# jason-gideon/GPUMounter

Measured on AMD Instinct MI355X. Metric: p50_gpu_attach_latency_ms, lower is better.
Workload: dtype none

## Files before the change

### gpumounter_amd/_native.py

```python
from __future__ import annotations

import ctypes as C
import os
import subprocess
import threading
from typing import Optional

LIB_DIR = os.path.join(os.path.dirname(os.path.abspath(__file__)), "_lib")
NATIVE_DIR = os.path.join(os.path.dirname(os.path.dirname(os.path.abspath(__file__))), "native")

_lock = threading.Lock()
_libs: dict = {}


class NativeError(RuntimeError):
    pass


def lib_path(name: str) -> str:
    return os.path.join(LIB_DIR, name)


def build(target: str = "all", quiet: bool = True) -> None:
    import fcntl
# ... 71 lines not shown
def mock_smi() -> C.CDLL:
    lib = _load("libamd_smi_mock.so", "host")
    lib.gm_mock_set_procs_file.argtypes = [C.c_char_p]
    lib.gm_mock_set_ecc.argtypes = [C.c_uint32, C.c_uint64, C.c_uint64]
    return lib


class DevRule(C.Structure):
    _fields_ = [("type", C.c_char), ("access", C.c_uint8), ("allow", C.c_uint8),
                ("pad", C.c_uint8), ("major", C.c_int32), ("minor", C.c_int32)]


class DevNode(C.Structure):
    _fields_ = [("path", C.c_char * 112), ("major", C.c_uint32), ("minor", C.c_uint32),
                ("mode", C.c_uint32), ("uid", C.c_int32), ("gid", C.c_int32)]


class BpfTiming(C.Structure):
    _fields_ = [("query_ns", C.c_uint64), ("map_ns", C.c_uint64), ("build_ns", C.c_uint64),
                ("load_ns", C.c_uint64), ("attach_ns", C.c_uint64), ("programs", C.c_uint32),
                ("insns", C.c_uint32)]


HOST_ABI_VERSION = 6
GM_ACC_MKNOD, GM_ACC_READ, GM_ACC_WRITE = 1, 2, 4
GM_DEV_EMULATE, GM_DEV_VIA_SETNS, GM_DEV_REPLACE, GM_DEV_BIND = 1, 2, 4, 8


def host() -> C.CDLL:
    lib = _load("libgm_host.so", "host")
    if not getattr(lib, "_gm_typed", False):
        abi = lib.gm_host_abi_version()
        if abi != HOST_ABI_VERSION:
            raise RuntimeError(f"libgm_host.so ABI {abi} != {HOST_ABI_VERSION} expected: stale "
                               f"build, run `make -C native`")
        lib.gm_cg1_apply.argtypes = [C.c_char_p, C.POINTER(DevRule), C.c_int]
        lib.gm_cg1_format_rule.argtypes = [C.POINTER(DevRule), C.c_char_p, C.c_int]
        lib.gm_bpf_dev_build.argtypes = [C.POINTER(DevRule), C.c_int, C.c_int, C.c_int,
                                         C.POINTER(C.c_uint64), C.c_int]
        lib.gm_bpf_dev_load.argtypes = [C.POINTER(C.c_uint64), C.c_int, C.c_char_p, C.c_char_p,
                                        C.c_int]
        lib.gm_bpf_dev_query.argtypes = [C.c_char_p, C.POINTER(C.c_uint32), C.c_uint32,
                                         C.POINTER(C.c_uint32), C.POINTER(C.c_uint32)]
        lib.gm_bpf_prog_name.argtypes = [C.c_uint32, C.c_char_p, C.c_int]
        lib.gm_bpf_dev_program.argtypes = [C.c_char_p, C.POINTER(C.c_uint64), C.c_uint32,
                                           C.POINTER(C.c_uint32), C.POINTER(C.c_uint32)]
        lib.gm_bpf_dev_program_at.argtypes = [C.c_char_p, C.c_uint32, C.c_int,
                                              C.POINTER(C.c_uint64),
                                              C.c_uint32, C.POINTER(C.c_uint32),
# ... 3 lines not shown
                                           C.POINTER(C.c_uint32), C.POINTER(C.c_uint32)]
        lib.gm_bpf_dev_restore.argtypes = [C.c_char_p, C.c_char_p]
        lib.gm_bpf_dev_build_set.argtypes = [C.c_int, C.POINTER(DevRule), C.c_int, C.c_int,
                                             C.c_int, C.POINTER(C.c_uint64), C.c_int]
        lib.gm_bpf_dev_probe_set.argtypes = []
        lib.gm_devnodes_bind_probe.argtypes = []
        lib.gm_bpf_dev_straight_line.argtypes = [C.c_int]
        lib.gm_bpf_dev_straight_line.restype = None
        lib.gm_bpf_dev_set_at.argtypes = [C.c_char_p, C.c_uint32, C.POINTER(C.c_uint32),
                                          C.c_uint32, C.POINTER(C.c_uint32),
                                          C.POINTER(C.c_uint32)]
        lib.gm_bpf_dev_last_timing.argtypes = [C.POINTER(BpfTiming)]
        lib.gm_bpf_dev_last_timing.restype = None
        lib.gm_devnodes_create.argtypes = [C.c_int, C.c_char_p, C.POINTER(DevNode), C.c_int,
                                           C.c_int, C.POINTER(C.c_int)]
        lib.gm_devnodes_remove.argtypes = lib.gm_devnodes_create.argtypes
        lib.gm_devnodes_guard.argtypes = [C.c_char_p]
        lib.gm_devnodes_stage.argtypes = [C.c_char_p, C.c_int]
        lib.gm_devnode_stat.argtypes = [C.c_int, C.c_char_p, C.c_char_p, C.c_int,
                                        C.POINTER(C.c_int), C.POINTER(C.c_uint32),
                                        C.POINTER(C.c_uint32), C.POINTER(C.c_uint32)]
        lib.gm_devnodes_present.argtypes = [C.c_int, C.c_char_p, C.POINTER(DevNode), C.c_int,
                                            C.c_int, C.POINTER(C.c_uint8)]
        lib.gm_proc_dev_users.argtypes = [C.c_uint32, C.c_uint32, C.POINTER(C.c_int32), C.c_int,
                                          C.POINTER(C.c_int)]
        lib.gm_proc_scan_devs.argtypes = [C.POINTER(C.c_int32), C.c_int, C.POINTER(C.c_uint32),
                                          C.c_int, C.POINTER(C.c_uint8), C.POINTER(C.c_int32)]
        lib.gm_proc_filter_dev_users.argtypes = [C.POINTER(C.c_int32), C.c_int, C.c_uint32,
                                                 C.c_uint32, C.POINTER(C.c_int32)]
        lib.gm_proc_read_pids.argtypes = [C.c_char_p, C.POINTER(C.c_int32), C.c_int,
                                          C.POINTER(C.c_int)]
        lib.gm_sd_get_device_allow.argtypes = [C.c_char_p, C.c_char_p, C.c_char_p, C.c_int,
                                               C.c_char_p, C.c_int]
        lib.gm_sd_set_device_allow.argtypes = [C.c_char_p, C.c_char_p, C.POINTER(C.c_char_p),
                                               C.POINTER(C.c_char_p), C.c_int, C.c_int,
                                               C.c_char_p, C.c_int]
        lib.gm_sd_unit_path.argtypes = [C.c_char_p, C.c_char_p, C.c_int]
        lib.gm_roctx_push.argtypes = [C.c_char_p]
        lib.gm_roctx_mark.argtypes = [C.c_char_p]
        lib.gm_roctx_start.argtypes = [C.c_char_p]
        lib.gm_roctx_start.restype = C.c_uint64
        lib.gm_roctx_stop.argtypes = [C.c_uint64]
        lib.gm_roctx_stop.restype = None
        lib.gm_now_ns.restype = C.c_uint64
        lib._gm_typed = True
    return lib
# ... 113 lines not shown
```

### gpumounter_amd/node/devnodes.py

```python
from __future__ import annotations

import ctypes as C
import errno
import os
from dataclasses import dataclass
from typing import List, Optional, Sequence, Tuple

from gpumounter_amd import _native
from gpumounter_amd.models.device import DeviceNode
from gpumounter_amd.utils import log


class DevNodeError(RuntimeError):
    def __init__(self, msg: str, results: Sequence[int] = ()):
        super().__init__(msg)
        self.results = list(results)


@dataclass(frozen=True)
class Target:

    pid: int = 0
    root: str = ""

# ... 6 lines not shown
class DevNodeWriter:

    def __init__(self, mode: str = "procroot", host_dev: str = "", userns: str = "auto",
                 stage_dir: str = "", proc_root: str = "/proc") -> None:
        self.mode = mode
        self.userns = userns
        self.stage_dir = stage_dir
        self.proc_root = proc_root
        self._staged = False
        self._own_userns = self._userns_id("self")
        self.flags = 0
        if mode == "setns":
            self.flags |= _native.GM_DEV_VIA_SETNS
        if mode == "emulate":
            self.flags |= _native.GM_DEV_EMULATE
        self.host_dev = host_dev
        rc = _native.host().gm_devnodes_guard(host_dev.encode() if host_dev else None)
        if rc < 0:
            _log.warning("host /dev guard off: cannot read %s (%s)", host_dev, os.strerror(-rc))
        self.guarded = max(rc, 0)

    @staticmethod
    def _array(nodes: Sequence[DeviceNode], owner: Tuple[int, int] = (-1, -1)):
        arr = (_native.DevNode * max(len(nodes), 1))()
        for i, n in enumerate(nodes):
            rel = n.path.lstrip("/").encode()
            if len(rel) >= 112:
                raise DevNodeError(f"path too long: {n.path}")
            arr[i].path = rel
            arr[i].major = n.major
            arr[i].minor = n.minor
            arr[i].mode = n.mode
            arr[i].uid, arr[i].gid = owner
        return arr

    def _mntns(self, pid) -> Optional[str]:
        try:
            return os.readlink(f"{self.proc_root}/{pid}/ns/mnt")
        except OSError:
            return None

    def root_pid(self, pids: Sequence[int]) -> int:
        if self.mode == "emulate":
            return pids[0] if pids else 0
        own = self._mntns("self")
        for pid in pids:
            ns = self._mntns(pid)
            if ns is not None and ns != own:
                return pid
        return 0

    def _userns_id(self, pid) -> Optional[Tuple[int, int]]:
        try:
            st = os.stat(f"{self.proc_root}/{pid}/ns/user")
        except OSError:
            return None
        return st.st_dev, st.st_ino
# ... 43 lines not shown
        if not self._bind(t):
            return self.flags, (-1, -1)
        self._ensure_stage()
        return self.flags | _native.GM_DEV_BIND, self._mapped_root(t)

    def _target_args(self, t: Target) -> Tuple[int, Optional[bytes]]:
        if t.root:
            return 0, t.root.encode()
        if t.pid <= 0:
            raise DevNodeError("container has no process to resolve its root from "
                               "(empty cgroup.procs)")
        return t.pid, None

    def create(self, t: Target, nodes: Sequence[DeviceNode]) -> List[int]:
        if not nodes:
            return []
        pid, root = self._target_args(t)
        flags, owner = self._call(t)
        res = (C.c_int * len(nodes))()
        fails = _native.host().gm_devnodes_create(pid, root, self._array(nodes, owner),
                                                  len(nodes), flags, res)
        results = [int(res[i]) for i in range(len(nodes))]
        if fails:
            bad = [(n.path, os.strerror(-r)) for n, r in zip(nodes, results) if r < 0]
            what = "bind mount" if flags & _native.GM_DEV_BIND else "mknod"
            raise DevNodeError(f"{what} failed: {bad}", results)
        return results

    def remove(self, t: Target, nodes: Sequence[DeviceNode]) -> List[int]:
        if not nodes:
            return []
        pid, root = self._target_args(t)
        flags, _ = self._call(t)
        res = (C.c_int * len(nodes))()
        fails = _native.host().gm_devnodes_remove(pid, root, self._array(nodes), len(nodes),
                                                  flags, res)
        results = [int(res[i]) for i in range(len(nodes))]
        if fails and not flags & _native.GM_DEV_BIND and \
                any(r == -errno.EBUSY for r in results) and self.mode != "emulate":
            busy = [i for i, r in enumerate(results) if r == -errno.EBUSY]
            self._ensure_stage()
            sub = [nodes[i] for i in busy]
            res2 = (C.c_int * len(sub))()
            _native.host().gm_devnodes_remove(pid, root, self._array(sub), len(sub),
                                              flags | _native.GM_DEV_BIND, res2)
            for k, i in enumerate(busy):
                results[i] = int(res2[k])
            fails = sum(1 for r in results if r < 0)
        if fails:
            if all(r in (-errno.ESRCH, -errno.ENOENT) for r in results if r < 0):
# ... 37 lines not shown
```

### gpumounter_amd/node/hotmount.py

```python
from __future__ import annotations

import os
from dataclasses import dataclass, field
from typing import Dict, List, Optional, Sequence

from gpumounter_amd.hw.inventory import Inventory
from gpumounter_amd.models.device import AmdGpu, DeviceNode, kfd_node
from gpumounter_amd.models.pod import ContainerRef, running_containers
from gpumounter_amd.node.cgroup import CgroupError, CgroupResolver, DeviceRuleBackend
from gpumounter_amd.node.devnodes import CREATED, DevNodeError, DevNodeWriter, Target
from gpumounter_amd.node.journal import InjectionJournal
from gpumounter_amd.utils import log, trace

_log = log.get("node.hotmount")


class MountError(RuntimeError):
    pass


@dataclass
class ContainerTarget:
    ref: ContainerRef
    cgdir: str
    target: Target
    pids: List[int] = field(default_factory=list)


@dataclass
class AuditIssue:
    container: str
    kind: str
    path: str
    major: int
    minor: int


class HotMount:
    def __init__(self, cfg, inv: Inventory, resolver: CgroupResolver, backend: DeviceRuleBackend,
                 writer: DevNodeWriter, faults=None,
                 journal: Optional[InjectionJournal] = None) -> None:
        from gpumounter_amd.utils.faults import NONE

        self.cfg = cfg
        self.inv = inv
        self.resolver = resolver
        self.backend = backend
        self.writer = writer
        self.faults = faults if faults is not None else NONE
        self.journal = journal if journal is not None else InjectionJournal()
        self.expected: Dict[str, object] = {}

    def _apply(self, cgdir: str, grant, revoke, desired) -> None:
        try:
            self.backend.apply(cgdir, grant, revoke, desired)
        finally:
            fp = getattr(self.backend, "fingerprint", None)
            self.expected[cgdir] = fp(cgdir) if fp is not None else None

    def kfd(self) -> DeviceNode:
        return kfd_node(self.inv.kfd_major)

    def gpu_nodes(self, gpus: Sequence[AmdGpu]) -> List[DeviceNode]:
        out: List[DeviceNode] = []
        for g in sorted(gpus, key=lambda g: g.index):
            out.extend(g.device_nodes(self.cfg.drm_major, self.cfg.inject_card_nodes,
                                      self.cfg.device_file_mode))
        return out

    def managed_nodes(self, hot: Sequence[AmdGpu], base: Sequence[AmdGpu]) -> List[DeviceNode]:
        base_keys = {(n.major, n.minor) for n in self.gpu_nodes(base)}
        nodes = [n for n in self.gpu_nodes(hot) if (n.major, n.minor) not in base_keys]
        if hot and not base:
            nodes.insert(0, self.kfd())
# ... 20 lines not shown

    def _owner(self, pod: dict, t: ContainerTarget) -> dict:
        md = pod.get("metadata", {})
        return {"namespace": md.get("namespace", ""), "pod": md.get("name", ""),
                "pod_uid": md.get("uid", ""), "container": t.ref.name, "cgdir": t.cgdir}

    def resolve(self, pod: dict, container: str = "",
                include_privileged: bool = False) -> List[ContainerTarget]:
        try:
            return self.targets(pod, container, include_privileged)
        except (CgroupError, OSError) as e:
            raise MountError(f"cannot resolve the pod's containers: {e}") from e

    def attach(self, pod: dict, new: Sequence[AmdGpu], have: Sequence[AmdGpu],
               base: Sequence[AmdGpu] = (), container: str = "") -> List[ContainerTarget]:
        before = self.managed_nodes(have, base)
        after = self.managed_nodes(list(have) + list(new), base)
        before_keys = {(n.major, n.minor) for n in before}
        grant = [n for n in after if (n.major, n.minor) not in before_keys]
        with trace.span("resolve"):
            targets = self.resolve(pod, container)
        done: List[tuple] = []
        j = self.journal
        try:
            for t in targets:
                cid = t.ref.id
                known = j.nodes_of(cid)
                with trace.span("devnodes_probe", nodes=len(after)):
                    states = self.writer.present_states(t.target, after)
                theirs = {(n.major, n.minor) for n, st in zip(after, states)
                          if st and (n.major, n.minor) not in known}
                j.intend(cid, [((n.major, n.minor), n.path) for n in grant],
                         [((n.major, n.minor), n.path) for n in after
                          if (n.major, n.minor) not in theirs], **self._owner(pod, t))
                done.append((t, grant, []))
                with trace.span("cgroup_rule", backend=self.backend.name, rules=len(grant)):
                    self.faults.check("cgroup_rule")
                    self._apply(t.cgdir, grant, [], after)
                self.faults.check("cgroup_rule", "after")
                with trace.span("devnodes", nodes=len(after)):
                    self.faults.check("devnodes")
                    res = self.writer.create(t.target, after)
                done[-1] = (t, grant, [n for n, r in zip(after, res) if r == CREATED])
                j.settle(cid, [(n.major, n.minor) for n, r in zip(after, res)
                               if r != CREATED and (n.major, n.minor) not in known
                               and (n.major, n.minor) not in theirs])
                self.faults.check("devnodes", "after")
        except Exception as e:
            self._rollback_attach(done, before)
            for t in targets[len(done):]:
                self._forget_new(t.ref.id, grant, after, before)
            raise MountError(f"attach failed, rolled back: {e}") from e
        return targets

    def _forget_new(self, cid: str, granted, after, before) -> None:
        keep = {(n.major, n.minor) for n in before}
        self.journal.forget(cid, [(n.major, n.minor) for n in granted],
                            [(n.major, n.minor) for n in after if (n.major, n.minor) not in keep])

    def _rollback_attach(self, done, before: List[DeviceNode]) -> None:
        before_keys = {(n.major, n.minor) for n in before}
        for t, granted, created in reversed(done):
            try:
                self.writer.remove(t.target, created)
            except Exception as e:
                _log.error("rollback unlink in %s failed: %s", t.ref.name, e)
            else:
                self.journal.forget(t.ref.id, (), [(n.major, n.minor) for n in created
                                                   if (n.major, n.minor) not in before_keys])
            try:
                try:
                    have = self.backend.installed(t.cgdir)
                    revoke = [n for n in granted if (n.major, n.minor) in have]
                except Exception:
                    revoke = list(granted)
                if revoke:
                    self._apply(t.cgdir, [], revoke, before)
            except Exception as e:
                _log.error("rollback revoke in %s failed: %s", t.cgdir, e)
            else:
                self.journal.forget(t.ref.id, [(n.major, n.minor) for n in granted])
            ent = self.journal.nodes_of(t.ref.id)
            self.journal.forget(t.ref.id, (), [k for k in ent if k not in before_keys])

    def detach(self, pod: dict, remove: Sequence[AmdGpu], keep: Sequence[AmdGpu],
               base: Sequence[AmdGpu] = (), container: str = "",
               targets: Optional[List[ContainerTarget]] = None) -> List[ContainerTarget]:
        before = self.managed_nodes(list(keep) + list(remove), base)
        after = self.managed_nodes(keep, base)
        after_keys = {(n.major, n.minor) for n in after}
        revoke = [n for n in before if (n.major, n.minor) not in after_keys]
        if targets is None:
            with trace.span("resolve"):
                targets = self.resolve(pod, container)
        try:
            self._detach(targets, revoke, after)
        except (CgroupError, DevNodeError, OSError) as e:
            raise MountError(f"detach failed: {e}") from e
        return targets

    def _detach(self, targets: List[ContainerTarget], revoke: List[DeviceNode],
                after: List[DeviceNode]) -> None:
        keys = [(n.major, n.minor) for n in revoke]
        for t in targets:
            with trace.span("cgroup_rule", backend=self.backend.name, rules=len(revoke)):
                self.faults.check("unmount")
                self._apply(t.cgdir, [], revoke, after)
            self.faults.check("unmount", "after")
            ours = self.journal.nodes_of(t.ref.id)
            unlink = [n for n in revoke if (n.major, n.minor) in ours]
            with trace.span("devnodes", nodes=len(unlink)):
                self.writer.remove(t.target, unlink)
            self.journal.forget(t.ref.id, keys, keys)

    def adopt(self, pod: dict, hot: Sequence[AmdGpu], base: Sequence[AmdGpu] = ()) -> int:
        want = self.managed_nodes(hot, base)
        if not want:
            return 0
        n = 0
        for t in self.targets(pod):
            if self.journal.get(t.ref.id) is not None:
                continue
            granted = self.backend.installed(t.cgdir)
            states = self.writer.present_states(t.target, want)
            rules = [((d.major, d.minor), d.path) for d in want if (d.major, d.minor) in granted]
            nodes = [((d.major, d.minor), d.path) for d, st in zip(want, states) if st == 1]
            if rules or nodes:
# ... 122 lines not shown
```

### gpumounter_amd/node/journal.py

```python
from __future__ import annotations

import json
import os
import threading
import time
from dataclasses import dataclass, field
from typing import Dict, Iterable, List, Optional, Tuple

from gpumounter_amd.utils import log

_log = log.get("node.journal")

Key = Tuple[int, int]


@dataclass
class Entry:
    container_id: str
    namespace: str = ""
    pod: str = ""
    pod_uid: str = ""
    container: str = ""
    cgdir: str = ""
    rules: Dict[Key, str] = field(default_factory=dict)
    nodes: Dict[Key, str] = field(default_factory=dict)
    updated: float = 0.0

    def empty(self) -> bool:
        return not self.rules and not self.nodes

    def to_json(self) -> dict:
        return {"container_id": self.container_id, "namespace": self.namespace, "pod": self.pod,
                "pod_uid": self.pod_uid, "container": self.container, "cgdir": self.cgdir,
                "rules": sorted([ma, mi, p] for (ma, mi), p in self.rules.items()),
                "nodes": sorted([ma, mi, p] for (ma, mi), p in self.nodes.items()),
                "updated": self.updated}
# ... 80 lines not shown
    def _entry(self, cid: str, owner: Optional[dict]) -> Entry:
        if not _safe_id(cid):
            raise ValueError(f"journal: bad container id {cid!r}")
        e = self._entries.get(cid)
        if e is None:
            e = self._entries[cid] = Entry(cid)
        if owner:
            for k, v in owner.items():
                if v:
                    setattr(e, k, v)
        return e

    def intend(self, cid: str, rules: Iterable[Tuple[Key, str]] = (),
               nodes: Iterable[Tuple[Key, str]] = (), **owner: str) -> None:
        with self._mu:
            e = self._entry(cid, owner)
            before = (len(e.rules), len(e.nodes))
            e.rules.update(rules)
            e.nodes.update(nodes)
            if (len(e.rules), len(e.nodes)) != before or not e.updated:
                e.updated = time.time()
                self._store(e)

    def settle(self, cid: str, not_ours: Iterable[Key]) -> None:
        keys = list(not_ours)
        if not keys:
            return
        with self._mu:
            e = self._entries.get(cid)
            if e is None:
                return
            changed = False
            for k in keys:
                changed |= e.nodes.pop(k, None) is not None
            if changed:
                e.updated = time.time()
                self._store(e)

    def forget(self, cid: str, rules: Iterable[Key] = (), nodes: Iterable[Key] = ()) -> None:
        with self._mu:
            e = self._entries.get(cid)
            if e is None:
                return
            changed = False
            for k in rules:
                changed |= e.rules.pop(k, None) is not None
# ... 16 lines not shown
```

### gpumounter_amd/utils/trace.py

```python
from __future__ import annotations

import contextvars
import os
import threading
import time
from dataclasses import dataclass, field
from typing import Callable, Dict, List, Optional

_current: contextvars.ContextVar[Optional["Span"]] = contextvars.ContextVar("gm_span", default=None)

_roctx_lock = threading.Lock()
_roctx = None
_sinks: List[Callable[["Span"], None]] = []


_names: Dict[str, bytes] = {}


def _profiled() -> bool:
    mode = os.environ.get("GM_ROCTX", "auto").lower()
    if mode in ("on", "1", "true"):
        return True
    if mode in ("off", "0", "false"):
        return False
# ... 83 lines not shown
        self.s.start_ns = time.perf_counter_ns()
        return self.s

    def __exit__(self, et, ev, tb):
        self.s.end_ns = time.perf_counter_ns()
        if ev is not None:
            self.s.error = f"{et.__name__}: {ev}"
        if self._lib is not None:
            self._lib.gm_roctx_stop(self._rid)
        _current.reset(self._tok)
        if self.s.parent is None:
            for fn in list(_sinks):
                try:
                    fn(self.s)
                except Exception:
                    pass
        return False


def current() -> Optional[Span]:
    return _current.get()


def record(name: str, duration_ns: int, **attrs) -> None:
    parent = _current.get()
    if parent is None or duration_ns <= 0:
        return
    start = parent.children[-1].end_ns if parent.children and parent.children[-1].end_ns \
        else parent.start_ns
    parent.children.append(Span(name=name, start_ns=start, end_ns=start + int(duration_ns),
                                attrs=attrs, parent=parent))


def annotate(**attrs) -> None:
    s = _current.get()
    if s is not None:
        s.attrs.update(attrs)


def mark(name: str) -> None:
    lib = _roctx_lib()
    if lib is not None:
        lib.gm_roctx_mark(name.encode())
```

### native/include/gm_host.h

```cpp
#pragma once
#include <stdint.h>

#ifdef __cplusplus
extern "C" {
#endif

#define GM_HOST_ABI_VERSION 6

#define GM_ACC_MKNOD 1
#define GM_ACC_READ 2
#define GM_ACC_WRITE 4

typedef struct gm_dev_rule {
  char type;
  uint8_t access;
  uint8_t allow;
  uint8_t pad;
  int32_t major;
  int32_t minor;
} gm_dev_rule_t;

int gm_cg1_apply(const char* cgdir, const gm_dev_rule_t* rules, int n);
int gm_cg1_format_rule(const gm_dev_rule_t* rule, char* out, int cap);

int gm_bpf_dev_build(const gm_dev_rule_t* rules, int n, int default_allow, int chain_map_fd,
                     uint64_t* out, int cap);
int gm_bpf_dev_build_set(int set_map_fd, const gm_dev_rule_t* base, int nbase, int default_allow,
                         int chain_map_fd, uint64_t* out, int cap);
int gm_bpf_dev_load(const uint64_t* insns, int n, const char* name, char* log, int logcap);
int gm_bpf_dev_query(const char* cgroup_path, uint32_t* ids, uint32_t cap, uint32_t* n,
// ... 24 lines not shown
  uint32_t minor;
  uint32_t mode;
  int32_t uid;
  int32_t gid;
} gm_dev_node_t;

#define GM_DEV_EMULATE 1
#define GM_DEV_VIA_SETNS 2
#define GM_DEV_REPLACE 4
#define GM_DEV_BIND 8

int gm_devnodes_guard(const char* host_dev);
int gm_devnodes_stage(const char* dir, int mount_tmpfs);
int gm_devnodes_bind_probe(void);
int gm_devnodes_create(int pid, const char* root, const gm_dev_node_t* nodes, int n, int flags,
                       int* results);
int gm_devnodes_remove(int pid, const char* root, const gm_dev_node_t* nodes, int n, int flags,
                       int* results);
int gm_devnode_stat(int pid, const char* root, const char* path, int flags, int* kind,
                    uint32_t* major, uint32_t* minor, uint32_t* mode);
int gm_devnodes_present(int pid, const char* root, const gm_dev_node_t* nodes, int n, int flags,
                        uint8_t* present);

int gm_proc_dev_users(uint32_t major, uint32_t minor, int32_t* pids, int cap, int* n);
int gm_proc_scan_devs(const int32_t* pids, int n, const uint32_t* majmin, int ndev,
                      uint8_t* hits, int32_t* unreadable);
int gm_proc_filter_dev_users(const int32_t* pids, int n, uint32_t major, uint32_t minor,
                             int32_t* out);
int gm_proc_read_pids(const char* path, int32_t* pids, int cap, int* n);

int gm_sd_get_device_allow(const char* bus_path, const char* unit, char* out, int cap, char* err,
                           int errcap);
int gm_sd_set_device_allow(const char* bus_path, const char* unit, const char* const* paths,
                           const char* const* perms, int n, int reset, char* err, int errcap);
int gm_sd_unit_path(const char* unit, char* out, int cap);

int gm_roctx_available(void);
void gm_roctx_push(const char* name);
void gm_roctx_pop(void);
void gm_roctx_mark(const char* name);
uint64_t gm_roctx_start(const char* name);
void gm_roctx_stop(uint64_t id);
uint64_t gm_now_ns(void);

int gm_host_abi_version(void);

// ... 4 lines not shown
```

### native/src/gm_host.cpp

```cpp
#include "gm_host.h"

#include <dirent.h>
#include <dlfcn.h>
#include <errno.h>
#include <fcntl.h>
#include <linux/bpf.h>
#include <sched.h>
#include <signal.h>
#include <stdio.h>
#include <stdlib.h>
#include <string.h>
#include <sys/mount.h>
#include <sys/stat.h>
#include <sys/syscall.h>
#include <sys/sysmacros.h>
#include <time.h>
#include <unistd.h>

#include <atomic>
#include <map>
#include <mutex>
#include <string>
#include <thread>
#include <vector>
// ... 502 lines not shown
  }
  if (comps.empty()) return -EINVAL;
  int cur = dup(rootfd);
  if (cur < 0) return -errno;
  Fd curfd(cur);
  for (size_t i = 0; i + 1 < comps.size(); ++i) {
    int nfd = openat(curfd.fd, comps[i].c_str(), O_PATH | O_DIRECTORY | O_NOFOLLOW | O_CLOEXEC);
    if (nfd < 0 && errno == ENOENT && create) {
      if (guarded_dir(curfd.fd)) return kSharedHost;
      if (mkdirat(curfd.fd, comps[i].c_str(), 0755) < 0 && errno != EEXIST) return -errno;
      nfd = openat(curfd.fd, comps[i].c_str(), O_PATH | O_DIRECTORY | O_NOFOLLOW | O_CLOEXEC);
    }
    if (nfd < 0) return -errno;
    curfd = Fd(nfd);
  }
  *leaf = comps.back();
  *parent = std::move(curfd);
  return 0;
}

struct Walker {
  int rootfd;
  bool mknod_denied = false;
  std::map<std::string, Fd> dirs;
  explicit Walker(int r) : rootfd(r) {}
  int parent(const char* path, bool create, int* dirfd, std::string* leaf) {
    std::string p(path);
    size_t cut = p.rfind('/');
    std::string dir = cut == std::string::npos ? std::string() : p.substr(0, cut);
    auto it = dirs.find(dir);
    if (it != dirs.end()) {
      *leaf = p.substr(cut + 1);
      if (leaf->empty() || *leaf == "." || *leaf == "..") return -EINVAL;
      *dirfd = it->second.fd;
      return 0;
    }
    Fd fd;
    int e = walk_parent(rootfd, path, create, &fd, leaf);
    if (e != 0) return e;
    *dirfd = fd.fd;
    dirs.emplace(dir, std::move(fd));
    return 0;
  }
};

int stat_leaf(int dirfd, const std::string& leaf, int* kind, uint32_t* maj, uint32_t* min,
              uint32_t* mode) {
  struct stat st;
  *kind = 0;
  *maj = *min = *mode = 0;
  if (fstatat(dirfd, leaf.c_str(), &st, AT_SYMLINK_NOFOLLOW) < 0) {
    if (errno == ENOENT) return 0;
    return -errno;
  }
  *mode = st.st_mode & 07777;
  if (S_ISCHR(st.st_mode)) {
    *kind = 1;
    *maj = major(st.st_rdev);
    *min = minor(st.st_rdev);
    return 0;
  }
  *kind = 3;
// ... 841 lines not shown
  if (e < 0) {
    for (int i = 0; i < n; ++i) results[i] = e;
    return n;
  }
  return failures;
}

int gm_devnode_stat(int pid, const char* root, const char* path, int flags, int* kind,
                    uint32_t* maj, uint32_t* min, uint32_t* mode) {
  return with_root(pid, root, flags, [&](int rootfd) {
    Fd parent;
    std::string leaf;
    int e = walk_parent(rootfd, path, false, &parent, &leaf);
    if (e == -ENOENT) {
      *kind = 0;
      *maj = *min = *mode = 0;
      return 0;
    }
    if (e < 0) return e;
    return stat_leaf(parent.fd, leaf, kind, maj, min, mode);
  });
}

int gm_devnodes_present(int pid, const char* root, const gm_dev_node_t* nodes, int n, int flags,
                        uint8_t* present) {
  int count = 0;
  int e = with_root(pid, root, flags, [&](int rootfd) {
    Walker wk(rootfd);
    for (int i = 0; i < n; ++i) {
      present[i] = 0;
      int pfd;
      std::string leaf;
      int w = wk.parent(nodes[i].path, false, &pfd, &leaf);
      if (w == -ENOENT) {
        std::string dir(nodes[i].path);
        const size_t cut = dir.rfind('/');
        dir = cut == std::string::npos ? std::string() : dir.substr(0, cut);
        Fd d2;
        std::string l2;
        if (!dir.empty() && walk_parent(rootfd, dir.c_str(), false, &d2, &l2) == 0 &&
            guarded_dir(d2.fd)) {
          present[i] = kSharedHost;
          ++count;
        }
        continue;
      }
      if (w < 0) continue;
      if (guarded_dir(pfd)) {
        present[i] = kSharedHost;
        ++count;
        continue;
      }
      int kind = 0;
      uint32_t ma = 0, mi = 0, mode = 0;
      if (stat_leaf(pfd, leaf, &kind, &ma, &mi, &mode) < 0) continue;
      if ((kind == 1 || kind == 2) && ma == nodes[i].major && mi == nodes[i].minor &&
          (!(flags & GM_DEV_BIND) || is_mount_leaf(pfd, leaf) == 1)) {
        present[i] = 1;
        ++count;
      }
    }
    return 0;
  });
  return e < 0 ? e : count;
}

namespace {
bool pid_uses_dev(long pid, dev_t want) {
  char p[64];
  snprintf(p, sizeof(p), "/proc/%ld/fd", pid);
  int dfd = open(p, O_RDONLY | O_DIRECTORY | O_CLOEXEC);
  if (dfd < 0) return false;
  DIR* fds = fdopendir(dfd);
  if (!fds) {
    close(dfd);
    return false;
  }
  struct dirent* fe;
  bool hit = false;
  while (!hit && (fe = readdir(fds)) != nullptr) {
    if (fe->d_name[0] == '.') continue;
    struct stat st;
    if (fstatat(dirfd(fds), fe->d_name, &st, 0) == 0 && S_ISCHR(st.st_mode) && st.st_rdev == want)
      hit = true;
  }
  closedir(fds);
  return hit;
// ... 110 lines not shown
```

Baseline: 1.091.

## Fuse attach/detach probe, journal, cgroup rule and node creation into one native transaction

Result: no change. 1.101 (+1.0%).

```diff
diff --git a/gpumounter_amd/_native.py b/gpumounter_amd/_native.py
--- a/gpumounter_amd/_native.py
+++ b/gpumounter_amd/_native.py
@@ -117,9 +117,28 @@
                 ("insns", C.c_uint32)]
 
 
-HOST_ABI_VERSION = 6
+class Txn(C.Structure):
+    _fields_ = [("pid", C.c_int32), ("flags", C.c_int32), ("root", C.c_char_p),
+                ("desired", C.POINTER(DevNode)), ("known", C.POINTER(C.c_uint8)),
+                ("unlink", C.POINTER(DevNode)), ("n_desired", C.c_int32),
+                ("n_unlink", C.c_int32), ("cgdir", C.c_char_p), ("pin_dir", C.c_char_p),
+                ("base", C.POINTER(DevRule)), ("n_base", C.c_int32), ("backend", C.c_int32),
+                ("journal_path", C.c_char_p), ("record", C.c_char_p),
+                ("record_len", C.c_int32), ("fp_cap", C.c_int32),
+                ("states", C.POINTER(C.c_uint8)), ("results", C.POINTER(C.c_int32)),
+                ("fp", C.c_void_p), ("fp_len", C.c_int32), ("stage", C.c_int32),
+                ("err", C.c_int32), ("dir_walks", C.c_int32), ("prog_id", C.c_uint32),
+                ("chained_id", C.c_uint32), ("probe_ns", C.c_uint64),
+                ("journal_ns", C.c_uint64), ("rule_ns", C.c_uint64), ("nodes_ns", C.c_uint64)]
+
+
+HOST_ABI_VERSION = 7
 GM_ACC_MKNOD, GM_ACC_READ, GM_ACC_WRITE = 1, 2, 4
 GM_DEV_EMULATE, GM_DEV_VIA_SETNS, GM_DEV_REPLACE, GM_DEV_BIND = 1, 2, 4, 8
+GM_TXN_RECORDING, GM_TXN_BPF_SET = 1, 2
+(GM_TXN_ARGS, GM_TXN_PROBE, GM_TXN_JOURNAL, GM_TXN_RULE, GM_TXN_NODES,
+ GM_TXN_DONE) = range(6)
+GM_TXN_FOREIGN_NODE = 1
 
 
 def host() -> C.CDLL:
@@ -169,6 +188,8 @@
                                         C.POINTER(C.c_uint32), C.POINTER(C.c_uint32)]
         lib.gm_devnodes_present.argtypes = [C.c_int, C.c_char_p, C.POINTER(DevNode), C.c_int,
                                             C.c_int, C.POINTER(C.c_uint8)]
+        lib.gm_hotmount_attach.argtypes = [C.POINTER(Txn)]
+        lib.gm_hotmount_detach.argtypes = [C.POINTER(Txn)]
         lib.gm_proc_dev_users.argtypes = [C.c_uint32, C.c_uint32, C.POINTER(C.c_int32), C.c_int,
                                           C.POINTER(C.c_int)]
         lib.gm_proc_scan_devs.argtypes = [C.POINTER(C.c_int32), C.c_int, C.POINTER(C.c_uint32),
diff --git a/gpumounter_amd/node/devnodes.py b/gpumounter_amd/node/devnodes.py
--- a/gpumounter_amd/node/devnodes.py
+++ b/gpumounter_amd/node/devnodes.py
@@ -52,17 +52,14 @@
 
     @staticmethod
     def _array(nodes: Sequence[DeviceNode], owner: Tuple[int, int] = (-1, -1)):
-        arr = (_native.DevNode * max(len(nodes), 1))()
-        for i, n in enumerate(nodes):
+        uid, gid = owner
+        init = []
+        for n in nodes:
             rel = n.path.lstrip("/").encode()
             if len(rel) >= 112:
                 raise DevNodeError(f"path too long: {n.path}")
-            arr[i].path = rel
-            arr[i].major = n.major
-            arr[i].minor = n.minor
-            arr[i].mode = n.mode
-            arr[i].uid, arr[i].gid = owner
-        return arr
+            init.append((rel, n.major, n.minor, n.mode, uid, gid))
+        return (_native.DevNode * max(len(nodes), 1))(*init)
 
     def _mntns(self, pid) -> Optional[str]:
         try:
@@ -152,10 +149,15 @@
                                                   len(nodes), flags, res)
         results = [int(res[i]) for i in range(len(nodes))]
         if fails:
-            bad = [(n.path, os.strerror(-r)) for n, r in zip(nodes, results) if r < 0]
-            what = "bind mount" if flags & _native.GM_DEV_BIND else "mknod"
-            raise DevNodeError(f"{what} failed: {bad}", results)
+            raise self.create_error(nodes, results, flags)
         return results
+
+    @staticmethod
+    def create_error(nodes: Sequence[DeviceNode], results: Sequence[int],
+                     flags: int = 0) -> DevNodeError:
+        bad = [(n.path, os.strerror(-r)) for n, r in zip(nodes, results) if r < 0]
+        what = "bind mount" if flags & _native.GM_DEV_BIND else "mknod"
+        return DevNodeError(f"{what} failed: {bad}", results)
 
     def remove(self, t: Target, nodes: Sequence[DeviceNode]) -> List[int]:
         if not nodes:
diff --git a/gpumounter_amd/node/hotmount.py b/gpumounter_amd/node/hotmount.py
--- a/gpumounter_amd/node/hotmount.py
+++ b/gpumounter_amd/node/hotmount.py
@@ -1,14 +1,20 @@
 from __future__ import annotations
 
+import ctypes as C
+import errno
 import os
 from dataclasses import dataclass, field
 from typing import Dict, List, Optional, Sequence
 
+from gpumounter_amd import _native
 from gpumounter_amd.hw.inventory import Inventory
 from gpumounter_amd.models.device import AmdGpu, DeviceNode, kfd_node
 from gpumounter_amd.models.pod import ContainerRef, running_containers
-from gpumounter_amd.node.cgroup import CgroupError, CgroupResolver, DeviceRuleBackend
-from gpumounter_amd.node.devnodes import CREATED, DevNodeError, DevNodeWriter, Target
+from gpumounter_amd.node.cgroup import (BPF_STATE, CgroupError, CgroupResolver,
+                                        DeviceRuleBackend, V2BpfBackend, V2RecordingBackend,
+                                        _rule_array, oci_default_rules)
+from gpumounter_amd.node.devnodes import (CREATED, SHARED_HOST, DevNodeError, DevNodeWriter,
+                                          Target)
 from gpumounter_amd.node.journal import InjectionJournal
 from gpumounter_amd.utils import log, trace
 
@@ -50,6 +56,8 @@
         self.faults = faults if faults is not None else NONE
         self.journal = journal if journal is not None else InjectionJournal()
         self.expected: Dict[str, object] = {}
+        self.txn_counts: Dict[str, int] = {"fused": 0, "stepwise": 0}
+        self._txn_base = None
 
     def _apply(self, cgdir: str, grant, revoke, desired) -> None:
         try:
@@ -116,8 +124,12 @@
             targets = self.resolve(pod, container)
         done: List[tuple] = []
         j = self.journal
+        arr = self._txn_nodes(after) if self._fusable() else None
         try:
             for t in targets:
+                if arr is not None and self._attach_fused(pod, t, grant, after, arr, done):
+                    continue
+                self.txn_counts["stepwise"] += 1
                 cid = t.ref.id
                 known = j.nodes_of(cid)
                 with trace.span("devnodes_probe", nodes=len(after)):
@@ -152,6 +164,173 @@
         self.journal.forget(cid, [(n.major, n.minor) for n in granted],
                             [(n.major, n.minor) for n in after if (n.major, n.minor) not in keep])
 
+    _WRITER_STEPS = frozenset(("present_states", "create", "remove"))
+    _BACKEND_STEPS = frozenset(("apply", "fingerprint"))
+    _JOURNAL_STEPS = frozenset(("intend", "settle", "forget", "nodes_of"))
+
+    def _fusable(self) -> bool:
+        if self.faults:
+            return False
+        b, w, j = self.backend, self.writer, self.journal
+        if not (type(b) is V2RecordingBackend or (type(b) is V2BpfBackend and b.set_mode)):
+            return False
+        if type(w) is not DevNodeWriter or w.mode not in ("procroot", "emulate") \
+                or type(j) is not InjectionJournal:
+            return False
+        return self._WRITER_STEPS.isdisjoint(vars(w)) and \
+            self._BACKEND_STEPS.isdisjoint(vars(b)) and self._JOURNAL_STEPS.isdisjoint(vars(j))
+
+    def _txn_nodes(self, nodes: Sequence[DeviceNode]):
+        if any(n.path[:1] != "/" or n.path[1:2] == "/" for n in nodes):
+            return None
+        try:
+            return self.writer._array(nodes)
+        except DevNodeError:
+            return None
+
+    def _txn(self, t: ContainerTarget, after: Sequence[DeviceNode], arr, touch_root: bool):
+        w = self.writer
+        x = _native.Txn()
+        x.flags = w.flags
+        if touch_root:
+            try:
+                x.pid, x.root = w._target_args(t.target)
+                x.flags = w._call(t.target)[0]
+            except DevNodeError:
+                return None
+            if x.flags & _native.GM_DEV_BIND:
+                return None
+        n = len(after)
+        x.desired, x.n_desired = arr, n
+        x.cgdir = t.cgdir.encode()
+        if type(self.backend) is V2RecordingBackend:
+            x.backend = _native.GM_TXN_RECORDING
+            cap = 2048 + 192 * n
+        else:
+            x.backend = _native.GM_TXN_BPF_SET
+            x.pin_dir = self.backend.pin_dir.encode() if self.backend.pin_dir else None
+            if self._txn_base is None:
+                base = oci_default_rules()
+                self._txn_base = (_rule_array(base), len(base))
+            x.base, x.n_base = self._txn_base
+            cap = 64
+        x._fp = C.create_string_buffer(cap)
+        x.fp, x.fp_cap = C.addressof(x._fp), cap
+        j = self.journal
+        x.journal_path = j._path(t.ref.id).encode() if j.dir else None
+        return x
+
+    def _txn_rule_effects(self, x, cgdir: str, rules: int,
+                          desired: Sequence[DeviceNode]) -> None:
+        b = self.backend
+        ok = x.stage > _native.GM_TXN_RULE
+        b._installed.pop(cgdir, None)
+        if x.backend == _native.GM_TXN_RECORDING:
+            fp = C.string_at(x.fp, x.fp_len) if x.fp_len >= 0 else None
+            if ok and desired and fp is not None:
+                b._installed[cgdir] = (fp, frozenset((d.major, d.minor) for d in desired))
+        else:
+            fp = None if x.fp_len < 0 else \
+                tuple(C.cast(x.fp, C.POINTER(C.c_uint32))[i] for i in range(x.fp_len // 4))
+        self.expected[cgdir] = fp
+        sp = trace.record("cgroup_rule", x.rule_ns, backend=b.name, rules=rules)
+        if x.backend == _native.GM_TXN_BPF_SET and ok and desired:
+            if sp is not None:
+                tm = _native.BpfTiming()
+                _native.host().gm_bpf_dev_last_timing(C.byref(tm))
+                trace.record("bpf_query", tm.query_ns, sp)
+                trace.record("bpf_build", tm.build_ns, sp, insns=tm.insns)
+                trace.record("bpf_load_verify", tm.load_ns, sp, programs=tm.programs)
+                trace.record("bpf_chain_map", tm.map_ns, sp)
+                trace.record("bpf_attach", tm.attach_ns, sp)
+            log.kv(_log, 10, "bpf program installed", cgroup=cgdir, prog_id=x.prog_id,
+                   chained=x.chained_id, rules=x.n_desired)
+
+    def _txn_rule_error(self, x, cgdir: str) -> Exception:
+        msg = os.strerror(-x.err)
+        if x.backend == _native.GM_TXN_RECORDING:
+            return OSError(-x.err, msg, os.path.join(cgdir, BPF_STATE))
+        what = "install" if x.n_desired else "restore"
+        return CgroupError(f"bpf {what} on {cgdir}: {msg}")
+
+    def _attach_fused(self, pod: dict, t: ContainerTarget, grant: List[DeviceNode],
+                      after: List[DeviceNode], arr, done: List[tuple]) -> bool:
+        n = len(after)
+        x = self._txn(t, after, arr, touch_root=n > 0)
+        if x is None:
+            return False
+        j = self.journal
+        cid = t.ref.id
+        known = j.nodes_of(cid)
+        ent, blob = j.stage_intend(cid, [((d.major, d.minor), d.path) for d in grant],
+                                   [((d.major, d.minor), d.path) for d in after],
+                                   **self._owner(pod, t))
+        x.record, x.record_len = blob, len(blob or b"")
+        x._known = (C.c_uint8 * max(n, 1))(*[(d.major, d.minor) in known for d in after])
+        x._states = (C.c_uint8 * max(n, 1))()
+        x._results = (C.c_int32 * max(n, 1))()
+        x.known, x.states, x.results = x._known, x._states, x._results
+        rc = _native.host().gm_hotmount_attach(C.byref(x))
+        if rc == _native.GM_TXN_FOREIGN_NODE or x.stage == _native.GM_TXN_ARGS \
+                or (x.stage == _native.GM_TXN_RULE and x.err == -errno.ENOSPC):
+            return False
+        self.txn_counts["fused"] += 1
+        if x.stage == _native.GM_TXN_PROBE:
+            raise DevNodeError(f"read-back of {n} nodes: {os.strerror(-x.err)}")
+        trace.record("devnodes_probe", x.probe_ns, nodes=n)
+        j.adopt(ent, blob is not None, keep_empty=True)
+        if x.stage == _native.GM_TXN_JOURNAL:
+            raise OSError(-x.err, os.strerror(-x.err), j._path(cid))
+        done.append((t, grant, []))
+        self._txn_rule_effects(x, t.cgdir, len(grant), after)
+        if x.stage == _native.GM_TXN_RULE:
+            raise self._txn_rule_error(x, t.cgdir)
+        trace.record("devnodes", x.nodes_ns, nodes=n)
+        res = [int(x._results[i]) for i in range(n)]
+        if x.stage == _native.GM_TXN_NODES:
+            raise self.writer.create_error(after, res, x.flags)
+        done[-1] = (t, grant, [d for d, r in zip(after, res) if r == CREATED])
+        j.settle(cid, [(d.major, d.minor) for d, r in zip(after, res)
+                       if r != CREATED and (d.major, d.minor) not in known])
+        return True
+
+    def _detach_fused(self, t: ContainerTarget, revoke: List[DeviceNode],
+                      after: List[DeviceNode], arr, keys: List[tuple]) -> bool:
+        j = self.journal
+        cid = t.ref.id
+        ours = j.nodes_of(cid)
+        unlink = [d for d in revoke if (d.major, d.minor) in ours]
+        uarr = self._txn_nodes(unlink)
+        x = self._txn(t, after, arr, touch_root=bool(unlink)) if uarr is not None else None
+        if x is None:
+            return False
+        ent, blob = j.stage_forget(cid, keys, keys)
+        x.record, x.record_len = blob, len(blob or b"")
+        x._unlink, x._results = uarr, (C.c_int32 * max(len(unlink), 1))()
+        x.unlink, x.n_unlink, x.results = uarr, len(unlink), x._results
+        _native.host().gm_hotmount_detach(C.byref(x))
+        if x.stage == _native.GM_TXN_ARGS \
+                or (x.stage == _native.GM_TXN_RULE and x.err == -errno.ENOSPC):
+            return False
+        self.txn_counts["fused"] += 1
+        self._txn_rule_effects(x, t.cgdir, len(revoke), after)
+        if x.stage == _native.GM_TXN_RULE:
+            raise self._txn_rule_error(x, t.cgdir)
+        if x.stage == _native.GM_TXN_NODES:
+            with trace.span("devnodes", nodes=len(unlink)):
+                self.writer.remove(t.target, unlink)
+            j.forget(cid, keys, keys)
+            return True
+        trace.record("devnodes", x.nodes_ns, nodes=len(unlink))
+        shared = [d.path for d, r in zip(unlink, x._results) if r == SHARED_HOST]
+        if shared:
+            _log.warning("not unlinking %s: the container's directory is the host's /dev", shared)
+        if ent is not None:
+            j.adopt(ent, blob is not None, keep_empty=x.stage == _native.GM_TXN_JOURNAL)
+        if x.stage == _native.GM_TXN_JOURNAL:
+            raise OSError(-x.err, os.strerror(-x.err), j._path(cid))
+        return True
+
     def _rollback_attach(self, done, before: List[DeviceNode]) -> None:
         before_keys = {(n.major, n.minor) for n in before}
         for t, granted, created in reversed(done):
@@ -196,7 +375,11 @@
     def _detach(self, targets: List[ContainerTarget], revoke: List[DeviceNode],
                 after: List[DeviceNode]) -> None:
         keys = [(n.major, n.minor) for n in revoke]
+        arr = self._txn_nodes(after) if self._fusable() else None
         for t in targets:
+            if arr is not None and self._detach_fused(t, revoke, after, arr, keys):
+                continue
+            self.txn_counts["stepwise"] += 1
             with trace.span("cgroup_rule", backend=self.backend.name, rules=len(revoke)):
                 self.faults.check("unmount")
                 self._apply(t.cgdir, [], revoke, after)
diff --git a/gpumounter_amd/node/journal.py b/gpumounter_amd/node/journal.py
--- a/gpumounter_amd/node/journal.py
+++ b/gpumounter_amd/node/journal.py
@@ -12,6 +12,8 @@
 _log = log.get("node.journal")
 
 Key = Tuple[int, int]
+
+_ENCODE = json.JSONEncoder(separators=(",", ":")).encode
 
 
 @dataclass
@@ -138,6 +140,58 @@
                 e.updated = time.time()
                 self._store(e)
 
+    @staticmethod
+    def _blob(e: Entry) -> bytes:
+        return b"" if e.empty() else _ENCODE(e.to_json()).encode()
+
+    def stage_intend(self, cid: str, rules: Iterable[Tuple[Key, str]] = (),
+                     nodes: Iterable[Tuple[Key, str]] = (),
+                     **owner: str) -> Tuple[Entry, Optional[bytes]]:
+        if not _safe_id(cid):
+            raise ValueError(f"journal: bad container id {cid!r}")
+        with self._mu:
+            old = self._entries.get(cid)
+            e = Entry(cid) if old is None else \
+                Entry(cid, old.namespace, old.pod, old.pod_uid, old.container, old.cgdir,
+                      dict(old.rules), dict(old.nodes), old.updated)
+        for k, v in owner.items():
+            if v:
+                setattr(e, k, v)
+        before = (len(e.rules), len(e.nodes))
+        e.rules.update(rules)
+        e.nodes.update(nodes)
+        if (len(e.rules), len(e.nodes)) == before and e.updated:
+            return e, None
+        e.updated = time.time()
+        return e, self._blob(e)
+
+    def stage_forget(self, cid: str, rules: Iterable[Key] = (),
+                     nodes: Iterable[Key] = ()) -> Tuple[Optional[Entry], Optional[bytes]]:
+        with self._mu:
+            old = self._entries.get(cid)
+            if old is None:
+                return None, None
+            e = Entry(cid, old.namespace, old.pod, old.pod_uid, old.container, old.cgdir,
+                      dict(old.rules), dict(old.nodes), old.updated)
+        changed = False
+        for k in rules:
+            changed |= e.rules.pop(k, None) is not None
+        for k in nodes:
+            changed |= e.nodes.pop(k, None) is not None
+        if not changed:
+            return e, None
+        e.updated = time.time()
+        return e, self._blob(e)
+
+    def adopt(self, e: Entry, stored: bool, keep_empty: bool) -> None:
+        with self._mu:
+            if stored:
+                self.writes += 1
+            if e.empty() and not keep_empty:
+                self._entries.pop(e.container_id, None)
+            else:
+                self._entries[e.container_id] = e
+
     def settle(self, cid: str, not_ours: Iterable[Key]) -> None:
         keys = list(not_ours)
         if not keys:
diff --git a/gpumounter_amd/utils/trace.py b/gpumounter_amd/utils/trace.py
--- a/gpumounter_amd/utils/trace.py
+++ b/gpumounter_amd/utils/trace.py
@@ -129,14 +129,17 @@
     return _current.get()
 
 
-def record(name: str, duration_ns: int, **attrs) -> None:
-    parent = _current.get()
+def record(name: str, duration_ns: int, parent: Optional[Span] = None, **attrs) -> Optional[Span]:
+    if parent is None:
+        parent = _current.get()
     if parent is None or duration_ns <= 0:
-        return
+        return None
     start = parent.children[-1].end_ns if parent.children and parent.children[-1].end_ns \
         else parent.start_ns
-    parent.children.append(Span(name=name, start_ns=start, end_ns=start + int(duration_ns),
-                                attrs=attrs, parent=parent))
+    s = Span(name=name, start_ns=start, end_ns=start + int(duration_ns), attrs=attrs,
+             parent=parent)
+    parent.children.append(s)
+    return s
 
 
 def annotate(**attrs) -> None:
diff --git a/native/include/gm_host.h b/native/include/gm_host.h
--- a/native/include/gm_host.h
+++ b/native/include/gm_host.h
@@ -5,7 +5,7 @@
 extern "C" {
 #endif
 
-#define GM_HOST_ABI_VERSION 6
+#define GM_HOST_ABI_VERSION 7
 
 #define GM_ACC_MKNOD 1
 #define GM_ACC_READ 2
@@ -76,6 +76,50 @@
 int gm_devnodes_present(int pid, const char* root, const gm_dev_node_t* nodes, int n, int flags,
                         uint8_t* present);
 
+#define GM_TXN_RECORDING 1
+#define GM_TXN_BPF_SET 2
+
+#define GM_TXN_ARGS 0
+#define GM_TXN_PROBE 1
+#define GM_TXN_JOURNAL 2
+#define GM_TXN_RULE 3
+#define GM_TXN_NODES 4
+#define GM_TXN_DONE 5
+
+#define GM_TXN_FOREIGN_NODE 1
+
+typedef struct gm_txn {
+  int32_t pid;
+  int32_t flags;
+  const char* root;
+  const gm_dev_node_t* desired;
+  const uint8_t* known;
+  const gm_dev_node_t* unlink;
+  int32_t n_desired;
+  int32_t n_unlink;
+  const char* cgdir;
+  const char* pin_dir;
+  const gm_dev_rule_t* base;
+  int32_t n_base;
+  int32_t backend;
+  const char* journal_path;
+  const char* record;
+  int32_t record_len;
+  int32_t fp_cap;
+  uint8_t* states;
+  int32_t* results;
+  char* fp;
+  int32_t fp_len;
+  int32_t stage;
+  int32_t err;
+  int32_t dir_walks;
+  uint32_t prog_id, chained_id;
+  uint64_t probe_ns, journal_ns, rule_ns, nodes_ns;
+} gm_txn_t;
+
+int gm_hotmount_attach(gm_txn_t* t);
+int gm_hotmount_detach(gm_txn_t* t);
+
 int gm_proc_dev_users(uint32_t major, uint32_t minor, int32_t* pids, int cap, int* n);
 int gm_proc_scan_devs(const int32_t* pids, int n, const uint32_t* majmin, int ndev,
                       uint8_t* hits, int32_t* unreadable);
diff --git a/native/src/gm_host.cpp b/native/src/gm_host.cpp
--- a/native/src/gm_host.cpp
+++ b/native/src/gm_host.cpp
@@ -548,7 +548,9 @@
 struct Walker {
   int rootfd;
   bool mknod_denied = false;
+  int walks = 0;
   std::map<std::string, Fd> dirs;
+  std::map<std::string, int> absent;
   explicit Walker(int r) : rootfd(r) {}
   int parent(const char* path, bool create, int* dirfd, std::string* leaf) {
     std::string p(path);
@@ -561,9 +563,16 @@
       *dirfd = it->second.fd;
       return 0;
     }
+    if (!create) {
+      auto miss = absent.find(dir);
+      if (miss != absent.end()) return miss->second;
+    }
     Fd fd;
+    ++walks;
     int e = walk_parent(rootfd, path, create, &fd, leaf);
+    if (e == -ENOENT && !create) absent[dir] = e;
     if (e != 0) return e;
+    absent.erase(dir);
     *dirfd = fd.fd;
     dirs.emplace(dir, std::move(fd));
     return 0;
@@ -1451,47 +1460,296 @@
   });
 }
 
+namespace {
+int probe_nodes(Walker& wk, const gm_dev_node_t* nodes, int n, int flags, uint8_t* present) {
+  int count = 0;
+  for (int i = 0; i < n; ++i) {
+    present[i] = 0;
+    int pfd;
+    std::string leaf;
+    int w = wk.parent(nodes[i].path, false, &pfd, &leaf);
+    if (w == -ENOENT) {
+      std::string dir(nodes[i].path);
+      const size_t cut = dir.rfind('/');
+      dir = cut == std::string::npos ? std::string() : dir.substr(0, cut);
+      int d2;
+      std::string l2;
+      if (!dir.empty() && wk.parent(dir.c_str(), false, &d2, &l2) == 0 && guarded_dir(d2)) {
+        present[i] = kSharedHost;
+        ++count;
+      }
+      continue;
+    }
+    if (w < 0) continue;
+    if (guarded_dir(pfd)) {
+      present[i] = kSharedHost;
+      ++count;
+      continue;
+    }
+    int kind = 0;
+    uint32_t ma = 0, mi = 0, mode = 0;
+    if (stat_leaf(pfd, leaf, &kind, &ma, &mi, &mode) < 0) continue;
+    if ((kind == 1 || kind == 2) && ma == nodes[i].major && mi == nodes[i].minor &&
+        (!(flags & GM_DEV_BIND) || is_mount_leaf(pfd, leaf) == 1)) {
+      present[i] = 1;
+      ++count;
+    }
+  }
+  return count;
+}
+}
+
 int gm_devnodes_present(int pid, const char* root, const gm_dev_node_t* nodes, int n, int flags,
                         uint8_t* present) {
   int count = 0;
   int e = with_root(pid, root, flags, [&](int rootfd) {
     Walker wk(rootfd);
-    for (int i = 0; i < n; ++i) {
-      present[i] = 0;
-      int pfd;
-      std::string leaf;
-      int w = wk.parent(nodes[i].path, false, &pfd, &leaf);
-      if (w == -ENOENT) {
-        std::string dir(nodes[i].path);
-        const size_t cut = dir.rfind('/');
-        dir = cut == std::string::npos ? std::string() : dir.substr(0, cut);
-        Fd d2;
-        std::string l2;
-        if (!dir.empty() && walk_parent(rootfd, dir.c_str(), false, &d2, &l2) == 0 &&
-            guarded_dir(d2.fd)) {
-          present[i] = kSharedHost;
-          ++count;
-        }
-        continue;
-      }
-      if (w < 0) continue;
-      if (guarded_dir(pfd)) {
-        present[i] = kSharedHost;
-        ++count;
-        continue;
-      }
-      int kind = 0;
-      uint32_t ma = 0, mi = 0, mode = 0;
-      if (stat_leaf(pfd, leaf, &kind, &ma, &mi, &mode) < 0) continue;
-      if ((kind == 1 || kind == 2) && ma == nodes[i].major && mi == nodes[i].minor &&
-          (!(flags & GM_DEV_BIND) || is_mount_leaf(pfd, leaf) == 1)) {
-        present[i] = 1;
-        ++count;
-      }
-    }
+    count = probe_nodes(wk, nodes, n, flags, present);
     return 0;
   });
   return e < 0 ? e : count;
+}
+
+namespace {
+
+int txn_end(gm_txn_t* t, int stage, int err) {
+  t->stage = stage;
+  t->err = err;
+  return err;
+}
+
+bool json_plain(const char* s) {
+  for (; *s; ++s)
+    if (*s < 0x20 || *s > 0x7e || *s == '"' || *s == '\\') return false;
+  return true;
+}
+
+bool climbs(const char* path) {
+  const char* p = path;
+  while (*p) {
+    const char* e = strchr(p, '/');
+    const size_t len = e ? (size_t)(e - p) : strlen(p);
+    if (len == 2 && p[0] == '.' && p[1] == '.') return true;
+    if (!e) break;
+    p = e + 1;
+  }
+  return false;
+}
+
+int txn_check_nodes(const gm_dev_node_t* nodes, int n, bool recorded) {
+  if (n < 0 || (n > 0 && !nodes)) return -EINVAL;
+  for (int i = 0; i < n; ++i) {
+    const char* p = nodes[i].path;
+    if (!memchr(p, 0, sizeof(nodes[i].path)) || !*p || climbs(p)) return -EINVAL;
+    if (recorded && !json_plain(p)) return -EINVAL;
+  }
+  return 0;
+}
+
+int txn_check(const gm_txn_t* t) {
+  if (!t || !t->cgdir || !*t->cgdir) return -EINVAL;
+  if (t->backend != GM_TXN_RECORDING && t->backend != GM_TXN_BPF_SET) return -EINVAL;
+  if (t->flags & (GM_DEV_BIND | GM_DEV_VIA_SETNS)) return -EINVAL;
+  if (t->n_base < 0 || (t->n_base > 0 && !t->base)) return -EINVAL;
+  if (t->journal_path && t->record && t->record_len < 0) return -EINVAL;
+  if (t->fp_cap < 0 || (t->fp_cap > 0 && !t->fp)) return -EINVAL;
+  int e = txn_check_nodes(t->desired, t->n_desired, t->backend == GM_TXN_RECORDING);
+  return e ? e : txn_check_nodes(t->unlink, t->n_unlink, false);
+}
+
+int write_replace(const std::string& path, const char* data, size_t len, mode_t mode) {
+  const std::string tmp = path + ".tmp";
+  Fd fd(open(tmp.c_str(), O_WRONLY | O_CREAT | O_TRUNC | O_CLOEXEC, mode));
+  if (!fd.ok()) return -errno;
+  int e = write_all(fd.fd, data, len);
+  fd.reset();
+  if (e < 0) return e;
+  return rename(tmp.c_str(), path.c_str()) < 0 ? -errno : 0;
+}
+
+int txn_journal(const gm_txn_t* t) {
+  if (!t->journal_path || !*t->journal_path || !t->record) return 0;
+  if (t->record_len == 0) return unlink(t->journal_path) < 0 && errno != ENOENT ? -errno : 0;
+  return write_replace(t->journal_path, t->record, (size_t)t->record_len, 0600);
+}
+
+constexpr const char* kStateFile = "gm.bpf.json";
+
+const std::string& recorded_insns() {
+  static const std::string text = [] {
+    uint64_t prog[64];
+    int n = gm_bpf_dev_build_set(-2, nullptr, 0, 0, -2, prog, 64);
+    std::string s = "[";
+    for (int i = 0; i < n; ++i) {
+      char w[24];
+      snprintf(w, sizeof(w), "%s\"%016llx\"", i ? ", " : "", (unsigned long long)prog[i]);
+      s += w;
+    }
+    return s + "]";
+  }();
+  return text;
+}
+
+std::string recorded_state(const gm_dev_node_t* nodes, int n) {
+  std::string rules = "[", set = "[";
+  for (int i = 0; i < n; ++i) {
+    char b[192];
+    snprintf(b, sizeof(b), "%s[%u, %u, \"/%s\"]", i ? ", " : "", nodes[i].major, nodes[i].minor,
+             nodes[i].path);
+    rules += b;
+    snprintf(b, sizeof(b), "%s[%d, %u, %u, %d]", i ? ", " : "", BPF_DEVCG_DEV_CHAR,
+             nodes[i].major, nodes[i].minor, GM_ACC_READ | GM_ACC_WRITE);
+    set += b;
+  }
+  return "{\"rules\": " + rules + "], \"chained\": \"runtime-default\", \"mode\": \"set\", "
+         "\"set\": " + set + "], \"insns\": " + recorded_insns() + "}";
+}
+
+int txn_rules(gm_txn_t* t) {
+  int e = 0;
+  t->fp_len = -1;
+  const std::string cg(t->cgdir);
+  if (t->backend == GM_TXN_RECORDING) {
+    const std::string path = cg + "/" + kStateFile;
+    if (t->n_desired == 0) {
+      if (unlink(path.c_str()) < 0 && errno != ENOENT && errno != ENOTDIR) e = -errno;
+    } else {
+      const std::string blob = recorded_state(t->desired, t->n_desired);
+      if (blob.size() > (size_t)t->fp_cap) return -ENOSPC;
+      e = write_replace(path, blob.data(), blob.size(), 0666);
+    }
+    Fd fd(open(path.c_str(), O_RDONLY | O_CLOEXEC));
+    struct stat st;
+    if (fd.ok() && fstat(fd.fd, &st) == 0) {
+      if ((uint64_t)st.st_size > (uint64_t)t->fp_cap) return e < 0 ? e : -ENOSPC;
+      const size_t want = (size_t)st.st_size;
+      size_t got = 0;
+      while (got < want) {
+        ssize_t r = read(fd.fd, t->fp + got, want - got);
+        if (r < 0 && errno == EINTR) continue;
+        if (r <= 0) break;
+        got += (size_t)r;
+      }
+      if (got == want) t->fp_len = (int32_t)got;
+    }
+    return e;
+  }
+  if (t->n_desired == 0) {
+    e = gm_bpf_dev_restore(t->cgdir, t->pin_dir);
+  } else {
+    std::vector<gm_dev_rule_t> rules((size_t)t->n_desired);
+    for (int i = 0; i < t->n_desired; ++i)
+      rules[i] = gm_dev_rule_t{'c', GM_ACC_READ | GM_ACC_WRITE, 1, 0,
+                               (int32_t)t->desired[i].major, (int32_t)t->desired[i].minor};
+    uint32_t prog = 0, chained = 0;
+    e = gm_bpf_dev_install(t->cgdir, rules.data(), t->n_desired, t->base, t->n_base, t->pin_dir,
+                           &prog, &chained);
+    t->prog_id = prog;
+    t->chained_id = chained;
+  }
+  uint32_t ids[16], n = 0, flags = 0;
+  const uint32_t cap = (uint32_t)t->fp_cap / 4 < 16 ? (uint32_t)t->fp_cap / 4 : 16;
+  if (gm_bpf_dev_query(t->cgdir, ids, cap, &n, &flags) == 0) {
+    if (n > cap && cap < 16) return e < 0 ? e : -ENOSPC;
+    const uint32_t k = n < cap ? n : cap;
+    memcpy(t->fp, ids, k * 4);
+    t->fp_len = (int32_t)(k * 4);
+  }
+  return e < 0 ? e : 0;
+}
+
+}
+
+int gm_hotmount_attach(gm_txn_t* t) {
+  int e = txn_check(t);
+  if (e < 0) return t ? txn_end(t, GM_TXN_ARGS, e) : e;
+  const int n = t->n_desired;
+  if (n > 0 && (!t->states || !t->results)) return txn_end(t, GM_TXN_ARGS, -EINVAL);
+  t->probe_ns = t->journal_ns = t->rule_ns = t->nodes_ns = 0;
+  t->dir_walks = 0;
+  t->prog_id = t->chained_id = 0;
+  t->fp_len = -1;
+
+  uint64_t t0 = mono_ns();
+  Fd root;
+  if (n > 0) {
+    root = Fd(open_root(t->pid, t->root));
+    if (!root.ok()) return txn_end(t, GM_TXN_PROBE, root.fd);
+  }
+  Walker w(root.fd);
+  bool foreign = false;
+  if (n > 0) {
+    probe_nodes(w, t->desired, n, t->flags, t->states);
+    for (int i = 0; i < n; ++i) foreign |= t->states[i] && !(t->known && t->known[i]);
+  }
+  uint64_t t1 = mono_ns();
+  t->probe_ns = t1 - t0;
+  t->dir_walks = w.walks;
+  if (foreign) {
+    t->stage = GM_TXN_PROBE;
+    t->err = 0;
+    return GM_TXN_FOREIGN_NODE;
+  }
+
+  e = txn_journal(t);
+  uint64_t t2 = mono_ns();
+  t->journal_ns = t2 - t1;
+  if (e < 0) return txn_end(t, GM_TXN_JOURNAL, e);
+
+  e = txn_rules(t);
+  uint64_t t3 = mono_ns();
+  t->rule_ns = t3 - t2;
+  if (e < 0) return txn_end(t, GM_TXN_RULE, e);
+
+  int first = 0;
+  for (int i = 0; i < n; ++i) {
+    t->results[i] = create_one(w, t->desired[i], t->flags);
+    if (t->results[i] < 0 && !first) first = t->results[i];
+  }
+  t->nodes_ns = mono_ns() - t3;
+  t->dir_walks = w.walks;
+  if (first < 0) return txn_end(t, GM_TXN_NODES, first);
+  return txn_end(t, GM_TXN_DONE, 0);
+}
+
+int gm_hotmount_detach(gm_txn_t* t) {
+  int e = txn_check(t);
+  if (e < 0) return t ? txn_end(t, GM_TXN_ARGS, e) : e;
+  const int n = t->n_unlink;
+  if (n > 0 && !t->results) return txn_end(t, GM_TXN_ARGS, -EINVAL);
+  t->probe_ns = t->journal_ns = t->rule_ns = t->nodes_ns = 0;
+  t->dir_walks = 0;
+  t->prog_id = t->chained_id = 0;
+
+  uint64_t t0 = mono_ns();
+  e = txn_rules(t);
+  uint64_t t1 = mono_ns();
+  t->rule_ns = t1 - t0;
+  if (e < 0) return txn_end(t, GM_TXN_RULE, e);
+
+  int first = 0;
+  if (n > 0) {
+    Fd root(open_root(t->pid, t->root));
+    if (!root.ok()) {
+      for (int i = 0; i < n; ++i) t->results[i] = root.fd;
+      first = root.fd;
+    } else {
+      Walker w(root.fd);
+      for (int i = 0; i < n; ++i) {
+        t->results[i] = remove_one(w, t->unlink[i]);
+        if (t->results[i] < 0 && !first) first = t->results[i];
+      }
+      t->dir_walks = w.walks;
+    }
+  }
+  uint64_t t2 = mono_ns();
+  t->nodes_ns = t2 - t1;
+  if (first < 0) return txn_end(t, GM_TXN_NODES, first);
+
+  e = txn_journal(t);
+  t->journal_ns = mono_ns() - t2;
+  if (e < 0) return txn_end(t, GM_TXN_JOURNAL, e);
+  return txn_end(t, GM_TXN_DONE, 0);
 }
 
 namespace {
```
